# hzheng40/irbfn

Hardware: AMD Instinct MI355X
Metric: RBF-net evals/s (B queries x N centres), forward (higher is better)
Workload: dtype f32 (distances and Phi x W on f16 MFMA: exact fixed-point heads + float tails, hi/lo operand pairs; f32 accumulate)

## Files before the change

### irbfn_amd/csrc/abi.hip

```cpp
#include <new>
#include <string.h>

#include "common.h"
#include "rollout_step.h"

namespace irbfn {
thread_local int g_last_hip_error = 0;
int padded_D(int D);
}

using namespace irbfn;

static inline hipStream_t as_stream(void* s) { return reinterpret_cast<hipStream_t>(s); }

extern "C" {

int irbfn_abi_version(void) { return IRBFN_ABI_VERSION; }

int irbfn_last_hip_error(void) { return g_last_hip_error; }

int irbfn_device_count(void) {
  int n = 0;
  hipError_t e = hipGetDeviceCount(&n);
  if (e != hipSuccess) {
// ... 31 lines not shown
  if (DC < 0 || OP < 0) return IRBFN_ERR_UNSUPPORTED;
  for (int i = 0; i < n_ranges * nsplit; ++i)
    if (dim_ranges_host[i] < 0 || dim_ranges_host[i] >= max_ranges) return IRBFN_ERR_BAD_ARG;
  if (n_ranges > R) n_ranges = R;

  irbfn_net* net = new (std::nothrow) irbfn_net();
  if (!net) return IRBFN_ERR_BAD_ARG;
  memset(net, 0, sizeof(*net));
  net->D = D; net->R = R; net->K = K; net->O = O; net->basis = basis;
  net->bclass = basis_class(basis);
  net->DC = DC; net->OP = OP; net->N = R * K;
  net->S = (DC + 1 + OP + 3) & ~3;
  net->nsplit = nsplit; net->max_ranges = max_ranges > 0 ? max_ranges : 1; net->n_ranges = n_ranges;
  net->opt[IRBFN_OPT_FWD_F16_TERMS] = 3;
  net->opt[IRBFN_OPT_TICK_FUSED] = 1;

  const size_t tab = (size_t)(nsplit > 0 ? nsplit : 1) * net->max_ranges;
  const size_t nr = (size_t)(n_ranges > 0 ? n_ranges : 1) * (nsplit > 0 ? nsplit : 1);
  hipError_t e = hipSuccess;
  auto alloc = [&](void** p, size_t bytes) {
    if (e == hipSuccess) e = hipMalloc(p, bytes ? bytes : 4);
  };
  alloc((void**)&net->rec, (size_t)net->N * net->S * sizeof(float));
  alloc((void**)&net->bias, (size_t)OP * sizeof(float));
  alloc((void**)&net->sig2, (size_t)net->N * sizeof(float));
  net->Npad = (net->N + 15) & ~15;
  if (mfma_eligible(net)) alloc((void**)&net->recm, (size_t)net->Npad * mfma_record_floats(D, O) * sizeof(float));
  if (f16_eligible(net)) {
    alloc((void**)&net->f16_img, f16_image_bytes(net));
    alloc((void**)&net->f16_oscale, 128 * sizeof(float));
// ... 351 lines not shown
```

### irbfn_amd/csrc/common.h

```cpp
#pragma once

#include <hip/hip_runtime.h>
#include <stdint.h>

#include "irbfn_hip.h"

namespace irbfn {

constexpr int kWave = 64;
constexpr int kMaxSplit = 8;
constexpr int kMaxD = 8;
constexpr int kRedBlocks = 256;
constexpr int kSeedBlocksMax = 1024;

enum BasisClass : int { BC_GAUSS = 0, BC_IQ = 1, BC_IMQ = 2, BC_GENERIC = 3 };

inline int basis_class(int basis) {
  switch (basis) {
    case IRBFN_GAUSSIAN:
    case IRBFN_GAUSSIAN_WIDE:
    case IRBFN_GAUSSIAN_WIDER: return BC_GAUSS;
    case IRBFN_INVERSE_QUADRATIC: return BC_IQ;
    case IRBFN_INVERSE_MULTIQUADRIC: return BC_IMQ;
    default: return BC_GENERIC;
// ... 9 lines not shown
#define IRBFN_HIP_CHECK(expr)                         \
  do {                                                \
    hipError_t e__ = (expr);                          \
    if (e__ != hipSuccess) {                          \
      ::irbfn::g_last_hip_error = (int)e__;           \
      return IRBFN_ERR_HIP;                           \
    }                                                 \
  } while (0)

struct GateTables {
  const float* lo;
  const float* hi;
  const float* delta;
  const int* dim_ranges;
  int nsplit, max_ranges, n_ranges;
};

__host__ __device__ constexpr int mfma_cw(int D) { return (D + 1 + 3) & ~3; }

struct DynParams {
  float p[13];
};
struct DynParams64 {
  double p[13];
};
template <typename S> struct DynOf { using type = DynParams; };
template <> struct DynOf<double> { using type = DynParams64; };

}

// ... 14 lines not shown
  void* gram_hdr;
  int gram_ok;
  int gram_exp[5];
  int gram_checked;
  float* pack_part;
  int gamma_packed;
  int* vjp_flags;
  int vjp_gen;
  float* small_part;
  unsigned int* small_ticket;
  float* gate_lo;
  float* gate_hi;
  float* gate_delta;
  int* gate_ranges;
  int nsplit, max_ranges, n_ranges;
  float* sp_img;
  int sp_ok, sp_E, sp_cap, sp_RS, sp_EW, sp_OPS;
  float sp_mean_active;
  bool has_params;
  int opt[IRBFN_OPT_COUNT];
  char last_name[96];
  int last_grid, last_block;

  irbfn::GateTables gate() const {
    return irbfn::GateTables{gate_lo, gate_hi, gate_delta, gate_ranges, nsplit, max_ranges, n_ranges};
  }
};

namespace irbfn {
enum LaunchKind : int {
// ... 150 lines not shown
```

### irbfn_amd/csrc/rbf_forward.hip

```cpp
#include <math.h>
#include "rbf_forward.h"
#include "rollout_step.h"

#include <stdio.h>
#include <stdlib.h>
#include <string.h>

namespace irbfn {

int launch_forward_d3(const FwdArgs&, int, int, int, bool, bool, int, size_t, hipStream_t, int*);
int launch_forward_d4(const FwdArgs&, int, int, int, bool, bool, int, size_t, hipStream_t, int*);
int launch_forward_d7(const FwdArgs&, int, int, int, bool, bool, int, size_t, hipStream_t, int*);
int launch_forward_d8(const FwdArgs&, int, int, int, bool, bool, int, size_t, hipStream_t, int*);

static const int kCompiledOP[] = {2, 4, 5, 8, 10, 16, 32, 64, 100, 128};

int padded_O(int O) {
  for (int op : kCompiledOP)
    if (O <= op) return op;
  return -1;
}

int padded_D(int D) {
  if (D <= 3) return 3;
// ... 217 lines not shown

static void gram_wide_geometry(const irbfn_net* net, int64_t B, int* SW_out, int* QG_out) {
  const int nchunks = (net->N + 31) / 32;
  const long groups = (B + 31) / 32;
  int SW = 1;
  while (SW < 4 && (groups * SW + 7) / 8 < 256) SW *= 2;
  SW = opt_or(net, IRBFN_OPT_FWD_F16_S, SW);
  if (SW != 1 && SW != 2 && SW != 4) SW = 1;
  while (SW > 1 && (gram_wide_ring_bytes(net, SW) > 160 * 1024 || nchunks / SW < 2)) SW /= 2;
  int QG = groups <= 384 ? 2 : (SW == 1 ? 4 : 8 / SW);
  QG = opt_or(net, IRBFN_OPT_FWD_F16_QG, QG);
  if (QG < 1 || SW * QG > 8) QG = 8 / SW;
  *SW_out = SW; *QG_out = QG;
}

static bool plan_gram(const irbfn_net* net, int64_t B, LaunchPlan* p) {
  if (!net->f16_img || !gram_eligible(net)) return false;
  int S, QG;
  size_t lds;
  if (net->O > 16) {
    if ((net->DC != 7 && net->DC != 8) || net->O > 128) return false;
    gram_wide_geometry(net, B, &S, &QG);
    lds = gram_wide_lds_bytes(net, S, QG, 0);
    p->kind = LK_K1G_WIDE;
  } else {
    gram_geometry(net, B, (net->N + 31) / 32, &S, &QG);
    lds = gram_lds_bytes(S, QG, false);
    p->kind = LK_K1G;
  }
  if (lds > 160 * 1024) {
    p->kind = LK_NONE;
    return false;
  }
  p->status = IRBFN_OK;
  p->S = S; p->QG = QG; p->lds = lds;
  p->grid = (int)(((B + 31) / 32 + QG - 1) / QG); p->block = S * QG * 64;
  return true;
}

static LaunchPlan plan_forward(const irbfn_net* net, int64_t B) {
  LaunchPlan p;
// ... 190 lines not shown
  LaunchPlan p;
  if (!gram_gamma_eligible(net)) return p;
  const bool packed = net->gram_img && net->f16_img && (net->R == 1 || net->gamma_packed);
  if (!packed) { p.status = IRBFN_ERR_NO_PARAMS; return p; }
  if (!net->gram_ok) return p;
  const int nchunks = net->R * gram_gamma_cpr(net);
  int S, QG;
  gram_geometry(net, B, nchunks, &S, &QG);
  const int fs = net->opt[IRBFN_OPT_FWD_F16_S];
  if (fs > 0 && fs <= 7 && S != fs) {
    S = fs;
    QG = opt_or(net, IRBFN_OPT_FWD_F16_QG, 8 / S > 0 ? 8 / S : 1);
    if (S * QG > 16) QG = 1;
  }
  p.lds = gram_lds_bytes(S, QG, tick, true);
  if (p.lds > 160 * 1024) return p;
  p.kind = tick ? LK_TICK_K1G_GAMMA : LK_K1G_GAMMA; p.status = IRBFN_OK; p.mode = mode;
  p.S = S; p.QG = QG;
  p.grid = (int)(((B + 31) / 32 + QG - 1) / QG); p.block = S * QG * 64;
  return p;
}

int launch_forward_gamma(irbfn_net* net, const float* x, const float* gamma, float* out, int64_t B, hipStream_t s) {
  if (B == 0) return IRBFN_OK;
  if (net->opt[IRBFN_OPT_FWD_GAMMA_KERNEL] == IRBFN_FWDG_K1G) {
    const LaunchPlan g = plan_gram_gamma(net, B, false, -1);
    if (g.kind == LK_NONE) return g.status;
    const int rc = launch_forward_gram_gamma(net, g, x, gamma, out, B, s);
    if (rc == IRBFN_OK) record_launch(net, g);
    return rc;
  }
// ... 101 lines not shown
```

### irbfn_amd/csrc/rbf_forward_f16_narrow.h

```cpp
#pragma once

#include "rbf_forward_f16_wide.h"

namespace irbfn {

constexpr int kTickNarrowT = 8;
constexpr int kTickNarrowCP = 17;
constexpr int kTickNarrowSP = 65;

template <bool ROLL>
__device__ __forceinline__ void narrow_epilogue(const F16Args& a, const F16Roll& rl, int mode, unsigned char* lds, const f4_t (&acc)[2],
                                                const float (&gam)[2], int S, int slice, int qg, long q0, float inv_scale) {
  const int lane = threadIdx.x & 63;
  const int g = lane >> 4, n = lane & 15;
  __syncthreads();
  float* red = reinterpret_cast<float*>(lds);
  float* gl = red + (size_t)a.QG * S * 2 * 4 * 64;
  [[maybe_unused]] float* ctile = gl + a.QG * 32;
#pragma unroll
  for (int t = 0; t < 2; ++t)
#pragma unroll
    for (int r = 0; r < 4; ++r) red[(((qg * S + slice) * 2 + t) * 4 + r) * 64 + lane] = acc[t][r];
  if (slice == 0 && g == 0) { gl[qg * 32 + n] = gam[0]; gl[qg * 32 + 16 + n] = gam[1]; }
  __syncthreads();
  if (slice == 0 && n < a.O) {
    const float sc = a.oscale[n] * inv_scale;
    const float bi = a.bias[n];
#pragma unroll
    for (int t = 0; t < 2; ++t)
#pragma unroll
      for (int r = 0; r < 4; ++r) {
        float v = 0.0f;
        for (int s2 = 0; s2 < S; ++s2) v += red[(((qg * S + s2) * 2 + t) * 4 + r) * 64 + lane];
        const int row = t * 16 + 4 * g + r;
        const long q = q0 + row;
        float y = __builtin_fmaf(gl[qg * 32 + row] * v, sc, bi);
        if constexpr (ROLL) {
          if (rl.mirror != nullptr && n >= rl.T && q < a.B && rl.mirror[q] != 0) y = -y;
          ctile[(qg * 32 + row) * kTickNarrowCP + n] = y;
        }
        if (q < a.B && a.out != nullptr) a.out[q * a.O + n] = y;
      }
// ... 9 lines not shown
    float u[2 * kTickNarrowT];
    if (lane < 32) {
      const float* ur = ctile + (qg * 32 + lane) * kTickNarrowCP;
#pragma unroll
      for (int i = 0; i < 2 * kTickNarrowT; ++i) u[i] = ur[i];
    }
    asm volatile("s_waitcnt lgkmcnt(0)" ::: "memory");
    __builtin_amdgcn_wave_barrier();
    float* stage = ctile + (size_t)a.QG * 32 * kTickNarrowCP + (size_t)qg * 32 * kTickNarrowSP;
    if (lane < nvalid) {
      const long b = q0 + lane;
      float* o = stage + lane * kTickNarrowSP;
      auto ctl = [&](int i) {
        float v = u[0];
#pragma unroll
        for (int k = 1; k < 2 * kTickNarrowT; ++k) v = (i == k) ? u[k] : v;
        return v;
      };
      if (mode == IRBFN_ROLLOUT_ST_SELECT || mode == IRBFN_ROLLOUT_ST_KS) {
        float st[7];
#pragma unroll
        for (int i = 0; i < 7; ++i) st[i] = rl.state0[b * 7 + i];
        for (int t = 0; t < T; ++t) {
          if (mode == IRBFN_ROLLOUT_ST_SELECT) st_step<true>(st, ctl(t), ctl(T + t), rl.dp);
          else st_step<false>(st, ctl(t), ctl(T + t), rl.dp);
#pragma unroll
          for (int i = 0; i < 7; ++i) o[t * 7 + i] = st[i];
        }
      } else if (mode == IRBFN_ROLLOUT_FRENET_LS) {
        float st[8];
#pragma unroll
// ... 28 lines not shown
```

### irbfn_amd/csrc/rbf_forward_gram.h

```cpp
#pragma once

#include "rbf_forward_f16_narrow.h"

namespace irbfn {

typedef _Float16 h4_t __attribute__((ext_vector_type(4)));

constexpr int kGramHeadBytes = 2 * 64 * 8;
constexpr int kGramTailBytes = 2 * 2 * 64 * 16;
constexpr int kGramOpBytes = kGramHeadBytes + kGramTailBytes;
constexpr int gram_chunk_bytes(int NT = 1) { return kGramOpBytes + NT * 2 * kF16WBytes; }
constexpr int kGramChunkBytes = gram_chunk_bytes(1);
constexpr int kGramDims = 8;
#ifndef IRBFN_GRAM_RING
#define IRBFN_GRAM_RING 5
#endif
constexpr int kGramRing = IRBFN_GRAM_RING;
#ifndef IRBFN_GRAM_WAVES
#define IRBFN_GRAM_WAVES 4
#endif

struct GramHdr {
  float r[8];
  int ex, ec, eq, ea, e2;
// ... 15 lines not shown
  const int m = hf * 3 + (j - 5);
  return j < 5 ? GramSlot{1, 2 * g + hf, gram_comb_p(j), gram_comb_q(j)}
               : (g == 0 ? (m < 5 ? GramSlot{2, 0, gram_comb_p(m), gram_comb_q(m)} : GramSlot{3, 0, 2, 0})
                         : (g == 1 && hf == 0 && j == 5 ? GramSlot{3, 0, 3, 0} : GramSlot{0, 0, 0, 0}));
}
static_assert(kGramDims == 8, "four lane groups x two coordinates");
__host__ __device__ inline int gram_T(const GramHdr& h, const GramSlot sl) {
  return sl.kind == 1 ? h.ex + h.ec - 11 * (sl.p + sl.q) : (sl.kind == 2 ? h.eq + h.ea - 11 * (sl.p + sl.q) : h.e2 - 11 * sl.p);
}
__host__ __device__ inline int gram_ax(int T) { return (T + 1) >> 1; }

template <int BC>
__host__ __device__ constexpr float gram_phi_scale() { return BC == BC_IMQ ? 128.0f : kPhiScale; }

#ifdef IRBFN_GRAM_STAMPS
__device__ unsigned long long g_gram_stamps[32];
#define IRBFN_GRAM_T() __builtin_amdgcn_s_memtime()
#else
#define IRBFN_GRAM_T() 0ull
#endif

typedef float f2_t __attribute__((ext_vector_type(2)));
typedef unsigned u2_t __attribute__((ext_vector_type(2)));

__device__ __forceinline__ void split_pair_mix(float p0, float p1, unsigned& hi, unsigned& lo) {
  hi = __builtin_bit_cast(unsigned, __builtin_amdgcn_cvt_pkrtz(p0, p1));
  const float q0 = p0 * kLoGain, q1 = p1 * kLoGain;
  const float ng = -kLoGain;
  float d0, d1;
  asm("v_fma_mix_f32 %0, %1, %2, %3 op_sel:[0,0,0] op_sel_hi:[1,0,0]" : "=v"(d0) : "v"(hi), "s"(ng), "v"(q0));
  asm("v_fma_mix_f32 %0, %1, %2, %3 op_sel:[1,0,0] op_sel_hi:[1,0,0]" : "=v"(d1) : "v"(hi), "s"(ng), "v"(q1));
  lo = __builtin_bit_cast(unsigned, __builtin_amdgcn_cvt_pkrtz(d0, d1));
}

template <int BC>
// ... 7 lines not shown
                 "v"(u[T][1][2]), "v"(u[T][1][3]));
#define IRBFN_T8_TAIL0 ""
#define IRBFN_T8_TAIL1 "\n s_nop 7"
  if constexpr (BC == BC_GAUSS) { IRBFN_T8("v_exp_f32_e32", 0) IRBFN_T8("v_exp_f32_e32", 1) }
  else if constexpr (BC == BC_IQ) { IRBFN_T8("v_rcp_f32_e32", 0) IRBFN_T8("v_rcp_f32_e32", 1) }
  else { IRBFN_T8("v_rsq_f32_e32", 0) IRBFN_T8("v_rsq_f32_e32", 1) }
#undef IRBFN_T8
#undef IRBFN_T8_TAIL0
#undef IRBFN_T8_TAIL1
}

struct GramArgs {
  F16Args f;
  const unsigned char* __restrict__ gimg;
  const GramHdr* __restrict__ hdr;
};

__device__ __forceinline__ void gram_parts_f(float vh, float vl, float inv, float (&n)[3]) {
  const float a = vh * inv, b = vl * inv;
  n[0] = __builtin_rintf(a * 1024.0f) * (1.0f / 1024.0f);
  const float r1 = ((a - n[0]) + b) * 2048.0f;
  n[1] = (float)(_Float16)r1;
  const float r2 = (r1 - n[1]) * 2048.0f;
  n[2] = (float)(_Float16)r2;
}

template <int DC>
__device__ __forceinline__ bool gram_query_operands(const F16Args& a, const GramHdr* hp, const long (&qrow)[2], int g, h4_t (&bhd)[2],
                                                    h8_t (&btl)[2][2]) {
#pragma clang fp contract(off)
  static_assert(DC <= kGramDims, "eight coordinate slots");
  const int ex = hp->ex, ec = hp->ec, eq = hp->eq, ea = hp->ea, e2 = hp->e2;
  GramHdr hx;
  hx.ex = ex; hx.ec = ec; hx.eq = eq; hx.ea = ea; hx.e2 = e2;
  bool bad = hp->ok == 0;
  const float xinv = __builtin_ldexpf(1.0f, -ex), qinv = __builtin_ldexpf(1.0f, -eq);
  const float xlim = __builtin_ldexpf(1.0f, ex) * 0.999f, qlim = __builtin_ldexpf(1.0f, eq) * 0.999f;
  auto scale_of = [&](const GramSlot sl) -> float { return sl.kind == 0 ? 0.0f : __builtin_ldexpf(1.0f, gram_ax(gram_T(hx, sl))); };
  float rr[2];
#pragma unroll
  for (int c = 0; c < 2; ++c) rr[c] = (2 * g + c < DC) ? -hp->r[2 * g + c] : 0.0f;
#pragma unroll
  for (int t = 0; t < 2; ++t) {
    float nx[2][3], nq[3];
    float qh = 0.0f, ql = 0.0f;
#pragma unroll
    for (int c = 0; c < 2; ++c) {
      const int i = 2 * g + c;
      const float xv = (i < DC && i < a.Dreal) ? a.x[qrow[t] * a.Dreal + i] : 0.0f;
      const float sh = xv + rr[c];
      const float bb = sh - xv;
      const float sl = (xv - (sh - bb)) + (rr[c] - bb);
      bad = bad || !(__builtin_fabsf(sh) < xlim);
      gram_parts_f(sh, sl, xinv, nx[c]);
      const float ph = sh * sh;
      const float pl = __builtin_fmaf(sh, sh, -ph) + 2.0f * sh * sl;
      const float th = qh + ph;
      const float tb = th - qh;
      ql += ((qh - (th - tb)) + (ph - tb)) + pl;
      qh = th;
    }
#pragma unroll
    for (int off = 16; off <= 32; off *= 2) {
      const float oh = __shfl_xor(qh, off), ol = __shfl_xor(ql, off);
// ... 19 lines not shown
      for (int j = 0; j < 5; ++j) {
        const GramSlot sl = gram_tail_slot(32 * hf + j);
        btl[t][hf][j] = (_Float16)(nx[hf][sl.p] * scale_of(sl));
      }
#pragma unroll
      for (int j = 5; j < 8; ++j) {
        const GramSlot s0 = gram_tail_slot(32 * hf + j), s1 = gram_tail_slot(32 * hf + 8 + j);
        const float v0 = s0.kind == 2 ? nq[s0.p] * scale_of(s0) : scale_of(s0);
        const float v1 = scale_of(s1);
        btl[t][hf][j] = (_Float16)(g == 0 ? v0 : (g == 1 ? v1 : 0.0f));
      }
    }
  }
  return bad;
}
static_assert(gram_head_slot(0).kind == 1 && gram_head_slot(4 * 3 + 1).dim == 7 && gram_head_slot(2).kind == 2 && gram_head_slot(6).kind == 3 &&
              gram_head_slot(10).kind == 3 && gram_head_slot(10).p == 1 && gram_head_slot(14).kind == 0 && gram_head_slot(3).kind == 0, "head slots");
static_assert(gram_tail_slot(32 + 8 * 2 + 4).kind == 1 && gram_tail_slot(32 + 8 * 2 + 4).dim == 5 && gram_tail_slot(5).kind == 2 &&
              gram_tail_slot(32 + 6).kind == 2 && gram_tail_slot(32 + 7).kind == 3 && gram_tail_slot(32 + 7).p == 2 && gram_tail_slot(8 + 5).kind == 3 &&
              gram_tail_slot(8 + 5).p == 3 && gram_tail_slot(8 + 6).kind == 0 && gram_tail_slot(16 + 5).kind == 0 && gram_tail_slot(32 + 8 + 5).kind == 0, "tail slots");

__device__ __forceinline__ void gram_heads(const h4_t (&a)[2], const h4_t (&b)[2], f4_t (&u)[2][2]) {
  asm("v_mfma_f32_16x16x16_f16 %0, %4, %6, 0\n v_mfma_f32_16x16x16_f16 %1, %5, %6, 0\n v_mfma_f32_16x16x16_f16 %2, %4, %7, 0\n "
      "v_mfma_f32_16x16x16_f16 %3, %5, %7, 0\n s_nop 4"
      : "=&v"(u[0][0]), "=&v"(u[0][1]), "=&v"(u[1][0]), "=&v"(u[1][1])
      : "v"(a[0]), "v"(a[1]), "v"(b[0]), "v"(b[1]));
}
__device__ __forceinline__ void gram_heads2(const h4_t& a, const h4_t (&b)[2], f4_t (&u)[2]) {
  asm("v_mfma_f32_16x16x16_f16 %0, %2, %3, 0\n v_mfma_f32_16x16x16_f16 %1, %2, %4, 0\n s_nop 4"
      : "=&v"(u[0]), "=&v"(u[1])
// ... 39 lines not shown
      const float* rp = recs + ((j >> 2) * 16 + 4 * g + (j & 3)) * RF;
      float r2 = 0.0f;
#pragma unroll
      for (int d = 0; d < DC; ++d) {
        const float df = xq[d] - rp[d];
        r2 = __builtin_fmaf(df, df, r2);
      }
      if constexpr (FINITE_R2) r2 = r2 == __builtin_inff() ? 3.0e38f : r2;
      float arg = f16_arg<BC>(r2, rp[RF - 1]);
      if constexpr (BC == BC_IMQ) arg *= kPhiScale;
      t16[t * 8 + j] = arg;
    }
  }
}

void gram_fill_args(const irbfn_net* net, const float* x, float* out, int64_t B, int S, int QG, GramArgs* a);
int launch_forward_gram_wide(irbfn_net* net, const LaunchPlan& p, const float* x, float* out, int64_t B, hipStream_t s);

}
```

### irbfn_amd/csrc/rbf_forward_gram.hip

```cpp
#include <hip/hip_fp16.h>
#include <stdint.h>
#include <stdio.h>
#include <stdlib.h>

#include "rbf_forward_gram_body.h"

namespace irbfn {

template <int DC, int BC>
__global__ __launch_bounds__(1024, IRBFN_GRAM_WAVES) void rbf_fwd_f16gram(const GramArgs ga) {
  extern __shared__ __attribute__((aligned(16))) unsigned char lds[];
  gram_body<DC, BC, false>(ga, F16Roll{}, -1, lds);
}

template <int DC, int BC>
__global__ __launch_bounds__(1024, IRBFN_GRAM_WAVES) void rbf_tick_f16gram(const GramArgs ga, const F16Roll rl, const int mode) {
  extern __shared__ __attribute__((aligned(16))) unsigned char lds[];
  gram_body<DC, BC, true>(ga, rl, mode, lds);
}

static int gram_nt(const irbfn_net* net) { return (net->O + 15) / 16; }

bool gram_eligible(const irbfn_net* net) {
  return f16_eligible(net) && net->DC <= kGramDims;
}

size_t gram_image_bytes(const irbfn_net* net) {
  const int nchunks = (net->N + kF16Chunk - 1) / kF16Chunk;
  return (size_t)nchunks * gram_chunk_bytes(gram_nt(net));
}

size_t gram_header_bytes() { return sizeof(GramHdr); }

#ifdef IRBFN_GRAM_STAMPS
extern "C" int irbfn_debug_gram_stamps(unsigned long long* out32) {
  return (int)hipMemcpyFromSymbol(out32, HIP_SYMBOL(g_gram_stamps), sizeof(unsigned long long) * 32);
}
#endif

template <int DC>
static int launch_gram_bc(const GramArgs& a, int bc, int grid, int block, size_t lds, hipStream_t s) {
#define IRBFN_GCASE(BCV)                                                                                      \
  case BCV: {                                                                                                 \
    auto k = rbf_fwd_f16gram<DC, BCV>;                                                                        \
    if (lds > 48 * 1024) {                                                                                    \
      hipError_t e = hipFuncSetAttribute(reinterpret_cast<const void*>(k),                                    \
                                         hipFuncAttributeMaxDynamicSharedMemorySize, (int)lds);               \
      if (e != hipSuccess) { g_last_hip_error = (int)e; return IRBFN_ERR_HIP; }                               \
    }                                                                                                         \
    hipLaunchKernelGGL(k, dim3(grid), dim3(block), lds, s, a);                                                \
    break;                                                                                                    \
  }
  switch (bc) {
    IRBFN_GCASE(BC_GAUSS)
    IRBFN_GCASE(BC_IQ)
    IRBFN_GCASE(BC_IMQ)
    default: return IRBFN_ERR_UNSUPPORTED;
  }
#undef IRBFN_GCASE
  IRBFN_HIP_CHECK(hipGetLastError());
  return IRBFN_OK;
}

size_t gram_lds_bytes(int S, int QG, bool tick, bool gamma) {
  size_t ring = (size_t)S * kGramRing * kGramChunkBytes;
  if (gamma) ring += (size_t)S * QG * 128 * sizeof(float);
  size_t red = (size_t)S * QG * 2 * 4 * 64 + (size_t)QG * 32;
  if (tick) red += (size_t)QG * 32 * (kTickNarrowCP + kTickNarrowSP);
  red *= sizeof(float);
  return ring > red ? ring : red;
}

int launch_forward_gram(irbfn_net* net, const LaunchPlan& p, const float* x, float* out, int64_t B, hipStream_t s) {
  if (p.kind == LK_K1G_WIDE) return launch_forward_gram_wide(net, p, x, out, B, s);
  GramArgs a;
  gram_fill_args(net, x, out, B, p.S, p.QG, &a);
  switch (net->DC) {
    case 3: return launch_gram_bc<3>(a, net->bclass, p.grid, p.block, p.lds, s);
    case 4: return launch_gram_bc<4>(a, net->bclass, p.grid, p.block, p.lds, s);
    case 7: return launch_gram_bc<7>(a, net->bclass, p.grid, p.block, p.lds, s);
    case 8: return launch_gram_bc<8>(a, net->bclass, p.grid, p.block, p.lds, s);
    default: return IRBFN_ERR_UNSUPPORTED;
  }
}

template <int DC>
static int launch_tick_gram_bc(const GramArgs& a, const F16Roll& rl, int mode, int bc, int grid, int block, size_t lds, hipStream_t s) {
#define IRBFN_GCASE(BCV)                                                                                      \
  case BCV: {                                                                                                 \
    auto k = rbf_tick_f16gram<DC, BCV>;                                                                       \
    if (lds > 48 * 1024) {                                                                                    \
      hipError_t e = hipFuncSetAttribute(reinterpret_cast<const void*>(k),                                    \
                                         hipFuncAttributeMaxDynamicSharedMemorySize, (int)lds);               \
      if (e != hipSuccess) { g_last_hip_error = (int)e; return IRBFN_ERR_HIP; }                               \
    }                                                                                                         \
    hipLaunchKernelGGL(k, dim3(grid), dim3(block), lds, s, a, rl, mode);                                      \
    break;                                                                                                    \
  }
  switch (bc) {
    IRBFN_GCASE(BC_GAUSS)
    IRBFN_GCASE(BC_IQ)
    IRBFN_GCASE(BC_IMQ)
    default: return IRBFN_ERR_UNSUPPORTED;
  }
#undef IRBFN_GCASE
  IRBFN_HIP_CHECK(hipGetLastError());
  return IRBFN_OK;
}

int launch_tick_gram_narrow(irbfn_net* net, const LaunchPlan& p, const float* x, const int* mirror, const float* state0,
// ... 11 lines not shown
```

### irbfn_amd/csrc/rbf_forward_gram_body.h

```cpp
#pragma once

#include "rbf_forward_gram.h"

namespace irbfn {

struct GramGamma {
  const float* __restrict__ gamma;
  int R, cpr;
};

template <int DC, int BC, bool ROLL, bool GAMMA = false>
__device__ __forceinline__ void gram_body(const GramArgs& ga, const F16Roll& rl, int mode, unsigned char* lds,
                                          [[maybe_unused]] const GramGamma gm = GramGamma{nullptr, 1, 1}) {
  static_assert(DC <= kGramDims, "eight coordinate slots");
  const F16Args& a = ga.f;
  constexpr int CBL = f16_chunk_bytes(DC);
  constexpr int CB = kGramChunkBytes;
  const int tid = threadIdx.x, lane = tid & 63;
  const int wave = __builtin_amdgcn_readfirstlane(tid >> 6);
  const int S = a.S, QG = a.QG;
  const int slice = wave / QG, qg = wave % QG;
  const int g = lane >> 4, n = lane & 15;
  const long q0 = ((long)blockIdx.x * QG + qg) * 32;
  const GramHdr* hp = ga.hdr;
  long qrow[2];
#pragma unroll
  for (int t = 0; t < 2; ++t) {
    long q = q0 + t * 16 + n;
    q = q < a.B ? q : a.B - 1;
    qrow[t] = q < 0 ? 0 : q;
  }
  h4_t bhd[2];
  h8_t btl[2][2];
  const bool bad = gram_query_operands<DC>(a, hp, qrow, g, bhd, btl);
  const bool wave_bad = __builtin_amdgcn_ballot_w64(bad) != 0ull;

  const int c0 = (int)((long)a.nchunks * slice / S), c1 = (int)((long)a.nchunks * (slice + 1) / S);
  const int na = c1 - c0;
  int nsteps = 0;
  for (int s2 = 0; s2 < S; ++s2) {
    const int m = (int)((long)a.nchunks * (s2 + 1) / S) - (int)((long)a.nchunks * s2 / S);
    nsteps = m > nsteps ? m : nsteps;
  }
  unsigned char* ring = lds + (size_t)slice * kGramRing * CB;
  constexpr int NVI = CB / 1024;
  auto stage = [&](int k, int buf) {
    if (k >= na) return;
    const unsigned char* gp = ga.gimg + (size_t)(c0 + k) * CB + lane * 16;
    unsigned char* dst = ring + buf * CB;
    for (int v = qg; v < NVI; v += QG)
      __builtin_amdgcn_global_load_lds((gptr_t)(gp + v * 1024), (lptr_t)(dst + v * 1024), 16, 0, 0);
  };
  auto step_barrier = [&]() { asm volatile("s_waitcnt vmcnt(0) lgkmcnt(0)\n\ts_barrier" ::: "memory"); };
  auto next3 = [&](int b3) { return b3 == kGramRing - 1 ? 0 : b3 + 1; };
  constexpr int kGramPer = (kGramRing - 1) / 2;
  static_assert(kGramRing == 2 * kGramPer + 1 && kGramPer >= 1, "ring = 2 x (steps per barrier) + 1");
  [[maybe_unused]] float* gtile = nullptr;
  [[maybe_unused]] const float* grow = nullptr;
// ... 54 lines not shown
      unsigned wh[4], wl[4];
#pragma unroll
      for (int jj = 0; jj < 4; ++jj) split_pair_mix(t16[t * 8 + 2 * jj], t16[t * 8 + 2 * jj + 1], wh[jj], wl[jj]);
      const h8_t ah = __builtin_bit_cast(h8_t, u4_t{wh[0], wh[1], wh[2], wh[3]});
      const h8_t al = __builtin_bit_cast(h8_t, u4_t{wl[0], wl[1], wl[2], wl[3]});
      acc[t] = __builtin_amdgcn_mfma_f32_16x16x32_f16(ah, bh, acc[t], 0, 0, 0);
      acl[t] = __builtin_amdgcn_mfma_f32_16x16x32_f16(al, bh, acl[t], 0, 0, 0);
      acl[t] = __builtin_amdgcn_mfma_f32_16x16x32_f16(ah, bl, acl[t], 0, 0, 0);
    }
  };

#pragma unroll
  for (int k = 0; k <= kGramPer; ++k) stage(k, k);
  gamma_stage(0);
  step_barrier();
#pragma unroll
  for (int k = kGramPer + 1; k < kGramRing; ++k) stage(k, k);
  gamma_stage(1);
  if (!wave_bad) {
    f4_t ua[2][2], ub[2][2];
    if (na > 0) distances(ring, ua);
    asm volatile("s_nop 7\n\ts_nop 7" ::: "memory");
    int b0 = 0;
    [[maybe_unused]] unsigned long long tph[5] = {0, 0, 0, 0, 0};
    auto one_step = [&](int i, f4_t (&ucur)[2][2], f4_t (&unxt)[2][2]) {
      const int b1 = next3(b0);
      [[maybe_unused]] const unsigned long long t0 = IRBFN_GRAM_T();
      if (i + 1 < na) distances(ring + b1 * CB, unxt);
      if (i < na) {
        gamma_read(i);
        float t16[16];
        products(t16, ring + b0 * CB, [&](float (&o)[16]) { trans16<BC>(ucur, o); });
      }
      [[maybe_unused]] const unsigned long long t2 = IRBFN_GRAM_T();
      end_of_step(i, b0);
      [[maybe_unused]] const unsigned long long t4 = IRBFN_GRAM_T();
#ifdef IRBFN_GRAM_STAMPS
      tph[1] += t2 - t0; tph[2] += t4 - t2; tph[4] += 1;
#endif
      b0 = b1;
    };
    for (int i = 0; i < nsteps; i += 2) {
      one_step(i, ua, ub);
      if (i + 1 < nsteps) one_step(i + 1, ub, ua);
    }
#ifdef IRBFN_GRAM_STAMPS
    if (blockIdx.x < 2 && tid == 0)
      for (int k = 0; k < 5; ++k) g_gram_stamps[blockIdx.x * 8 + k] = tph[k];
#endif
  } else {
    int b0 = 0;
    for (int i = 0; i < nsteps; ++i) {
      if (i < na) {
        gamma_read(i);
        float t16[16];
        gram_valu_args<DC, BC, GAMMA>(a, qrow, g, reinterpret_cast<const float*>(a.img + (size_t)(c0 + i) * CBL), t16);
        products(t16, ring + b0 * CB, [&](float (&o)[16]) { trans_block<BC, 16>(o); });
      }
      end_of_step(i, b0);
      b0 = next3(b0);
    }
  }
#pragma unroll
  for (int t = 0; t < 2; ++t)
#pragma unroll
    for (int r = 0; r < 4; ++r) acc[t][r] = __builtin_fmaf(acl[t][r], kLoScale, acc[t][r]);

  const GateTables gt = a.gate;
  float gam[2] = {0.0f, 0.0f};
  if constexpr (GAMMA) {
    gam[0] = gam[1] = 1.0f;
  } else if (slice == 0) {
#pragma unroll
    for (int t = 0; t < 2; ++t) {
      float gv = gt.n_ranges > 0 ? 1.0f : 0.0f;
#pragma unroll
      for (int d = 0; d < DC; ++d)
        if (d < gt.nsplit && gt.n_ranges > 0) {
          const int e = d * gt.max_ranges + gt.dim_ranges[d];
          gv *= gate_factor(a.x[qrow[t] * a.Dreal + d], gt.lo[e], gt.hi[e], gt.delta[d]);
        }
      gam[t] = gv;
    }
  }
  narrow_epilogue<ROLL>(a, rl, mode, lds, acc, gam, S, slice, qg, q0, 1.0f / (gram_phi_scale<BC>() * kWScale));
}

}
```

### irbfn_amd/csrc/rbf_forward_gram_gamma.hip

```cpp
#ifdef IRBFN_GRAM_STAMPS
#undef IRBFN_GRAM_STAMPS
#endif
#include <hip/hip_fp16.h>
#include <stdint.h>

#include "rbf_forward_gram_body.h"

namespace irbfn {

template <int DC, int BC>
__global__ __launch_bounds__(1024, IRBFN_GRAM_WAVES) void rbf_fwd_f16gram_gamma(const GramArgs ga, const GramGamma gm) {
  extern __shared__ __attribute__((aligned(16))) unsigned char lds[];
  gram_body<DC, BC, false, true>(ga, F16Roll{}, -1, lds, gm);
}

template <int DC, int BC>
__global__ __launch_bounds__(1024, IRBFN_GRAM_WAVES) void rbf_tick_f16gram_gamma(const GramArgs ga, const GramGamma gm, const F16Roll rl,
                                                                                 const int mode) {
  extern __shared__ __attribute__((aligned(16))) unsigned char lds[];
  gram_body<DC, BC, true, true>(ga, rl, mode, lds, gm);
}

int gram_gamma_cpr(const irbfn_net* net) { return (net->K + kF16Chunk - 1) / kF16Chunk; }

// ... 17 lines not shown
  }
  net->f16_img = static_cast<unsigned char*>(bufs[0]);
  net->f16_oscale = static_cast<float*>(bufs[1]);
  net->gram_img = static_cast<unsigned char*>(bufs[2]);
  net->gram_hdr = bufs[3];
  net->pack_part = static_cast<float*>(bufs[4]);
  net->gamma_packed = 0;
  return IRBFN_OK;
}

static void gamma_fill_args(const irbfn_net* net, const float* x, const float* gamma, float* out, int64_t B, int S, int QG, GramArgs* a,
                            GramGamma* gm) {
  gram_fill_args(net, x, out, B, S, QG, a);
  gm->gamma = gamma; gm->R = net->R; gm->cpr = gram_gamma_cpr(net);
  a->f.nchunks = gm->R * gm->cpr;
}

template <typename K, typename... Args>
static int launch_gg(K k, int grid, int block, size_t lds, hipStream_t s, Args... args) {
  if (lds > 48 * 1024) {
    hipError_t e = hipFuncSetAttribute(reinterpret_cast<const void*>(k), hipFuncAttributeMaxDynamicSharedMemorySize, (int)lds);
    if (e != hipSuccess) { g_last_hip_error = (int)e; return IRBFN_ERR_HIP; }
  }
  hipLaunchKernelGGL(k, dim3(grid), dim3(block), lds, s, args...);
  IRBFN_HIP_CHECK(hipGetLastError());
  return IRBFN_OK;
}

template <int DC>
static int launch_gg_fwd(const GramArgs& a, const GramGamma& gm, int bc, const LaunchPlan& p, hipStream_t s) {
// ... 44 lines not shown
```

### irbfn_amd/csrc/rbf_forward_gram_wide.hip

```cpp
#include "rbf_forward_gram_wide.h"

namespace irbfn {

template <int DC, int BC, int NT>
__global__ __launch_bounds__(512) void rbf_fwd_f16gram_wide(const GramArgs ga) {
  extern __shared__ __attribute__((aligned(16))) unsigned char lds[];
  wide_gram_body<DC, BC, NT, -1>(ga, F16Roll{}, lds);
}

template <int DC, int NT>
static int launch_gw_bc(const GramArgs& a, int bc, int grid, int block, size_t lds, hipStream_t s) {
#define IRBFN_GWCASE(BCV)                                                                                     \
  case BCV: {                                                                                                 \
    auto k = rbf_fwd_f16gram_wide<DC, BCV, NT>;                                                                \
    if (lds > 48 * 1024) {                                                                                    \
      hipError_t e = hipFuncSetAttribute(reinterpret_cast<const void*>(k),                                    \
                                         hipFuncAttributeMaxDynamicSharedMemorySize, (int)lds);               \
      if (e != hipSuccess) { g_last_hip_error = (int)e; return IRBFN_ERR_HIP; }                               \
    }                                                                                                         \
    hipLaunchKernelGGL(k, dim3(grid), dim3(block), lds, s, a);                                                \
    break;                                                                                                    \
  }
  switch (bc) {
    IRBFN_GWCASE(BC_GAUSS)
// ... 2 lines not shown
    default: return IRBFN_ERR_UNSUPPORTED;
  }
#undef IRBFN_GWCASE
  IRBFN_HIP_CHECK(hipGetLastError());
  return IRBFN_OK;
}

size_t gram_wide_ring_bytes(const irbfn_net* net, int SW) { return (size_t)SW * 3 * gram_chunk_bytes((net->O + 15) / 16); }

size_t gram_wide_lds_bytes(const irbfn_net* net, int SW, int QG, size_t extra_red_floats) {
  const size_t ring = gram_wide_ring_bytes(net, SW);
  const size_t red = ((size_t)SW * QG * 2 * 4 * 64 + (size_t)QG * 32 + extra_red_floats) * sizeof(float);
  return ring > red ? ring : red;
}

void gram_fill_args(const irbfn_net* net, const float* x, float* out, int64_t B, int S, int QG, GramArgs* a) {
  const int nchunks = (net->N + kF16Chunk - 1) / kF16Chunk;
  a->f.x = x; a->f.img = net->f16_img; a->f.oscale = net->f16_oscale; a->f.bias = net->bias; a->f.out = out; a->f.gate = net->gate();
  a->f.B = (long)B; a->f.Dreal = net->D; a->f.O = net->O; a->f.nchunks = nchunks; a->f.S = S; a->f.QG = QG;
  a->gimg = net->gram_img;
  a->hdr = reinterpret_cast<const GramHdr*>(net->gram_hdr);
}

int launch_forward_gram_wide(irbfn_net* net, const LaunchPlan& p, const float* x, float* out, int64_t B, hipStream_t s) {
  const int NT = (net->O + 15) / 16;
  GramArgs a;
  gram_fill_args(net, x, out, B, p.S, p.QG, &a);
  int rc;
#define IRBFN_GW_NT(DCV)                                                                      \
  switch (NT) {                                                                               \
    case 2: rc = launch_gw_bc<DCV, 2>(a, net->bclass, p.grid, p.block, p.lds, s); break;      \
    case 3: rc = launch_gw_bc<DCV, 3>(a, net->bclass, p.grid, p.block, p.lds, s); break;      \
    case 4: rc = launch_gw_bc<DCV, 4>(a, net->bclass, p.grid, p.block, p.lds, s); break;      \
    case 5: rc = launch_gw_bc<DCV, 5>(a, net->bclass, p.grid, p.block, p.lds, s); break;      \
    case 6: rc = launch_gw_bc<DCV, 6>(a, net->bclass, p.grid, p.block, p.lds, s); break;      \
    case 7: rc = launch_gw_bc<DCV, 7>(a, net->bclass, p.grid, p.block, p.lds, s); break;      \
// ... 10 lines not shown
```

Measured before the change: 827.4 million.

## Hoist gram kernel prologue work: precomputed gate row, nsteps, early loads, cached LDS attr

The host now resolves the per-dimension gate bounds into a flat GateRow and precomputes nsteps, passing both as kernel arguments. That replaces the dependent global-table lookups and the per-thread loop over slices. Query and radius loads are issued early, and slice 0 computes the gate and parks it in LDS before the main loop, so the epilogue no longer waits on global reads. Other changes: an unrolled compare replaces an integer divide, bias/oscale loads move before the epilogue barrier, and the hipFuncSetAttribute call is cached per device. The cost is extra LDS for the parked gate values, a gate0 snapshot that ignores later changes to the dim_ranges table, and phase timestamp probes under a debug define.

Result: faster. 844.3 million, median of 6 (+2.0%).

```diff
diff --git a/irbfn_amd/csrc/abi.hip b/irbfn_amd/csrc/abi.hip
--- a/irbfn_amd/csrc/abi.hip
+++ b/irbfn_amd/csrc/abi.hip
@@ -69,6 +69,13 @@
   net->nsplit = nsplit; net->max_ranges = max_ranges > 0 ? max_ranges : 1; net->n_ranges = n_ranges;
   net->opt[IRBFN_OPT_FWD_F16_TERMS] = 3;
   net->opt[IRBFN_OPT_TICK_FUSED] = 1;
+
+  net->gate0.nsplit = nsplit; net->gate0.n_ranges = n_ranges;
+  if (nsplit > 0 && n_ranges > 0)
+    for (int d = 0; d < nsplit; ++d) {
+      const int e = d * net->max_ranges + dim_ranges_host[d];
+      net->gate0.lo[d] = lo_tab_host[e]; net->gate0.hi[d] = hi_tab_host[e]; net->gate0.delta[d] = delta_host[d];
+    }
 
   const size_t tab = (size_t)(nsplit > 0 ? nsplit : 1) * net->max_ranges;
   const size_t nr = (size_t)(n_ranges > 0 ? n_ranges : 1) * (nsplit > 0 ? nsplit : 1);
diff --git a/irbfn_amd/csrc/common.h b/irbfn_amd/csrc/common.h
--- a/irbfn_amd/csrc/common.h
+++ b/irbfn_amd/csrc/common.h
@@ -47,6 +47,11 @@
   const float* delta;
   const int* dim_ranges;
   int nsplit, max_ranges, n_ranges;
+};
+
+struct GateRow {
+  float lo[kMaxSplit], hi[kMaxSplit], delta[kMaxSplit];
+  int nsplit, n_ranges;
 };
 
 __host__ __device__ constexpr int mfma_cw(int D) { return (D + 1 + 3) & ~3; }
@@ -91,6 +96,7 @@
   float* gate_delta;
   int* gate_ranges;
   int nsplit, max_ranges, n_ranges;
+  irbfn::GateRow gate0;
   float* sp_img;
   int sp_ok, sp_E, sp_cap, sp_RS, sp_EW, sp_OPS;
   float sp_mean_active;
diff --git a/irbfn_amd/csrc/rbf_forward.hip b/irbfn_amd/csrc/rbf_forward.hip
--- a/irbfn_amd/csrc/rbf_forward.hip
+++ b/irbfn_amd/csrc/rbf_forward.hip
@@ -255,6 +255,8 @@
   *SW_out = SW; *QG_out = QG;
 }
 
+static bool gram_slices_fit(int nchunks, int S) { return (long)nchunks * S < (1L << 31); }
+
 static bool plan_gram(const irbfn_net* net, int64_t B, LaunchPlan* p) {
   if (!net->f16_img || !gram_eligible(net)) return false;
   int S, QG;
@@ -266,6 +268,7 @@
     p->kind = LK_K1G_WIDE;
   } else {
     gram_geometry(net, B, (net->N + 31) / 32, &S, &QG);
+    if (!gram_slices_fit((net->N + 31) / 32, S)) return false;
     lds = gram_lds_bytes(S, QG, false);
     p->kind = LK_K1G;
   }
@@ -486,7 +489,7 @@
     if (S * QG > 16) QG = 1;
   }
   p.lds = gram_lds_bytes(S, QG, tick, true);
-  if (p.lds > 160 * 1024) return p;
+  if (p.lds > 160 * 1024 || !gram_slices_fit(nchunks, S)) return p;
   p.kind = tick ? LK_TICK_K1G_GAMMA : LK_K1G_GAMMA; p.status = IRBFN_OK; p.mode = mode;
   p.S = S; p.QG = QG;
   p.grid = (int)(((B + 31) / 32 + QG - 1) / QG); p.block = S * QG * 64;
diff --git a/irbfn_amd/csrc/rbf_forward_f16_narrow.h b/irbfn_amd/csrc/rbf_forward_f16_narrow.h
--- a/irbfn_amd/csrc/rbf_forward_f16_narrow.h
+++ b/irbfn_amd/csrc/rbf_forward_f16_narrow.h
@@ -13,6 +13,11 @@
                                                 const float (&gam)[2], int S, int slice, int qg, long q0, float inv_scale) {
   const int lane = threadIdx.x & 63;
   const int g = lane >> 4, n = lane & 15;
+  float sc = 0.0f, bi = 0.0f;
+  if (slice == 0 && n < a.O) {
+    sc = a.oscale[n] * inv_scale;
+    bi = a.bias[n];
+  }
   __syncthreads();
   float* red = reinterpret_cast<float*>(lds);
   float* gl = red + (size_t)a.QG * S * 2 * 4 * 64;
@@ -24,8 +29,6 @@
   if (slice == 0 && g == 0) { gl[qg * 32 + n] = gam[0]; gl[qg * 32 + 16 + n] = gam[1]; }
   __syncthreads();
   if (slice == 0 && n < a.O) {
-    const float sc = a.oscale[n] * inv_scale;
-    const float bi = a.bias[n];
 #pragma unroll
     for (int t = 0; t < 2; ++t)
 #pragma unroll
@@ -65,7 +68,11 @@
       auto ctl = [&](int i) {
         float v = u[0];
 #pragma unroll
-        for (int k = 1; k < 2 * kTickNarrowT; ++k) v = (i == k) ? u[k] : v;
+        for (int k = 1; k < 2 * kTickNarrowT; ++k) {
+          float uk = u[k];
+          asm("" : "+v"(uk));
+          v = (i == k) ? uk : v;
+        }
         return v;
       };
       if (mode == IRBFN_ROLLOUT_ST_SELECT || mode == IRBFN_ROLLOUT_ST_KS) {
diff --git a/irbfn_amd/csrc/rbf_forward_gram.h b/irbfn_amd/csrc/rbf_forward_gram.h
--- a/irbfn_amd/csrc/rbf_forward_gram.h
+++ b/irbfn_amd/csrc/rbf_forward_gram.h
@@ -53,11 +53,21 @@
 __host__ __device__ constexpr float gram_phi_scale() { return BC == BC_IMQ ? 128.0f : kPhiScale; }
 
 #ifdef IRBFN_GRAM_STAMPS
-__device__ unsigned long long g_gram_stamps[32];
+__device__ unsigned long long g_gram_stamps[64];
 #define IRBFN_GRAM_T() __builtin_amdgcn_s_memtime()
+#define IRBFN_GRAM_PHASE(k)                                                                            \
+  do {                                                                                                 \
+    asm volatile("s_waitcnt vmcnt(0) lgkmcnt(0)" ::: "memory");                                        \
+    if (blockIdx.x < 2 && threadIdx.x == 0) {                                                          \
+      g_gram_stamps[blockIdx.x * 32 + 8 + (k)] = __builtin_amdgcn_s_memtime();                         \
+      if ((k) == 0 || (k) == 6) g_gram_stamps[blockIdx.x * 32 + 16 + (k) / 6] = __builtin_amdgcn_s_memrealtime(); \
+    }                                                                                                  \
+  } while (0)
 #else
 #define IRBFN_GRAM_T() 0ull
+#define IRBFN_GRAM_PHASE(k) do { } while (0)
 #endif
+enum GramPhase : int { GP_ENTRY = 0, GP_OPERANDS, GP_BARRIER1, GP_LOOP0, GP_LOOP1, GP_GATE, GP_STORED };
 
 typedef float f2_t __attribute__((ext_vector_type(2)));
 typedef unsigned u2_t __attribute__((ext_vector_type(2)));
@@ -95,6 +105,8 @@
   F16Args f;
   const unsigned char* __restrict__ gimg;
   const GramHdr* __restrict__ hdr;
+  GateRow g0;
+  int nsteps;
 };
 
 __device__ __forceinline__ void gram_parts_f(float vh, float vl, float inv, float (&n)[3]) {
@@ -107,8 +119,24 @@
 }
 
 template <int DC>
-__device__ __forceinline__ bool gram_query_operands(const F16Args& a, const GramHdr* hp, const long (&qrow)[2], int g, h4_t (&bhd)[2],
-                                                    h8_t (&btl)[2][2]) {
+__device__ __forceinline__ void gram_query_loads(const F16Args& a, const GramHdr* hp, const long (&qrow)[2], int g, float (&xv)[2][2],
+                                                 float (&rv)[2]) {
+#pragma unroll
+  for (int c = 0; c < 2; ++c) rv[c] = hp->r[2 * g + c];
+#pragma unroll
+  for (int t = 0; t < 2; ++t)
+#pragma unroll
+    for (int c = 0; c < 2; ++c) {
+      const int i = 2 * g + c;
+      const bool in = i < DC && i < a.Dreal;
+      const float v = a.x[qrow[t] * a.Dreal + (in ? i : 0)];
+      xv[t][c] = in ? v : 0.0f;
+    }
+}
+
+template <int DC>
+__device__ __forceinline__ bool gram_query_operands(const F16Args& a, const GramHdr* hp, const float (&xin)[2][2], const float (&rin)[2],
+                                                    int g, h4_t (&bhd)[2], h8_t (&btl)[2][2]) {
 #pragma clang fp contract(off)
   static_assert(DC <= kGramDims, "eight coordinate slots");
   const int ex = hp->ex, ec = hp->ec, eq = hp->eq, ea = hp->ea, e2 = hp->e2;
@@ -120,15 +148,16 @@
   auto scale_of = [&](const GramSlot sl) -> float { return sl.kind == 0 ? 0.0f : __builtin_ldexpf(1.0f, gram_ax(gram_T(hx, sl))); };
   float rr[2];
 #pragma unroll
-  for (int c = 0; c < 2; ++c) rr[c] = (2 * g + c < DC) ? -hp->r[2 * g + c] : 0.0f;
+  for (int c = 0; c < 2; ++c) {
+    rr[c] = (2 * g + c < DC) ? -rin[c] : 0.0f;
+  }
 #pragma unroll
   for (int t = 0; t < 2; ++t) {
     float nx[2][3], nq[3];
     float qh = 0.0f, ql = 0.0f;
 #pragma unroll
     for (int c = 0; c < 2; ++c) {
-      const int i = 2 * g + c;
-      const float xv = (i < DC && i < a.Dreal) ? a.x[qrow[t] * a.Dreal + i] : 0.0f;
+      const float xv = xin[t][c];
       const float sh = xv + rr[c];
       const float bb = sh - xv;
       const float sl = (xv - (sh - bb)) + (rr[c] - bb);
@@ -178,6 +207,13 @@
   }
   return bad;
 }
+template <int DC>
+__device__ __forceinline__ bool gram_query_operands(const F16Args& a, const GramHdr* hp, const long (&qrow)[2], int g, h4_t (&bhd)[2],
+                                                    h8_t (&btl)[2][2]) {
+  float xv[2][2], rv[2];
+  gram_query_loads<DC>(a, hp, qrow, g, xv, rv);
+  return gram_query_operands<DC>(a, hp, xv, rv, g, bhd, btl);
+}
 static_assert(gram_head_slot(0).kind == 1 && gram_head_slot(4 * 3 + 1).dim == 7 && gram_head_slot(2).kind == 2 && gram_head_slot(6).kind == 3 &&
               gram_head_slot(10).kind == 3 && gram_head_slot(10).p == 1 && gram_head_slot(14).kind == 0 && gram_head_slot(3).kind == 0, "head slots");
 static_assert(gram_tail_slot(32 + 8 * 2 + 4).kind == 1 && gram_tail_slot(32 + 8 * 2 + 4).dim == 5 && gram_tail_slot(5).kind == 2 &&
@@ -247,6 +283,7 @@
   }
 }
 
+int gram_nsteps(int nchunks, int S);
 void gram_fill_args(const irbfn_net* net, const float* x, float* out, int64_t B, int S, int QG, GramArgs* a);
 int launch_forward_gram_wide(irbfn_net* net, const LaunchPlan& p, const float* x, float* out, int64_t B, hipStream_t s);
 
diff --git a/irbfn_amd/csrc/rbf_forward_gram.hip b/irbfn_amd/csrc/rbf_forward_gram.hip
--- a/irbfn_amd/csrc/rbf_forward_gram.hip
+++ b/irbfn_amd/csrc/rbf_forward_gram.hip
@@ -3,9 +3,13 @@
 #include <stdio.h>
 #include <stdlib.h>
 
+#include <atomic>
+
 #include "rbf_forward_gram_body.h"
 
 namespace irbfn {
+
+constexpr int kMaxDevices = 64;
 
 template <int DC, int BC>
 __global__ __launch_bounds__(1024, IRBFN_GRAM_WAVES) void rbf_fwd_f16gram(const GramArgs ga) {
@@ -33,21 +37,29 @@
 size_t gram_header_bytes() { return sizeof(GramHdr); }
 
 #ifdef IRBFN_GRAM_STAMPS
-extern "C" int irbfn_debug_gram_stamps(unsigned long long* out32) {
-  return (int)hipMemcpyFromSymbol(out32, HIP_SYMBOL(g_gram_stamps), sizeof(unsigned long long) * 32);
+extern "C" int irbfn_debug_gram_stamps(unsigned long long* out64) {
+  return (int)hipMemcpyFromSymbol(out64, HIP_SYMBOL(g_gram_stamps), sizeof(unsigned long long) * 64);
 }
 #endif
+
+struct DynLdsSet { std::atomic<unsigned> bytes[kMaxDevices]; };
+static int ensure_dyn_lds(const void* kernel, size_t lds, DynLdsSet* set) {
+  if (lds <= 48 * 1024) return IRBFN_OK;
+  int dev = 0;
+  IRBFN_HIP_CHECK(hipGetDevice(&dev));
+  if (dev >= 0 && dev < kMaxDevices && set->bytes[dev].load(std::memory_order_relaxed) >= lds) return IRBFN_OK;
+  IRBFN_HIP_CHECK(hipFuncSetAttribute(kernel, hipFuncAttributeMaxDynamicSharedMemorySize, (int)lds));
+  if (dev >= 0 && dev < kMaxDevices) set->bytes[dev].store((unsigned)lds, std::memory_order_relaxed);
+  return IRBFN_OK;
+}
 
 template <int DC>
 static int launch_gram_bc(const GramArgs& a, int bc, int grid, int block, size_t lds, hipStream_t s) {
 #define IRBFN_GCASE(BCV)                                                                                      \
   case BCV: {                                                                                                 \
     auto k = rbf_fwd_f16gram<DC, BCV>;                                                                        \
-    if (lds > 48 * 1024) {                                                                                    \
-      hipError_t e = hipFuncSetAttribute(reinterpret_cast<const void*>(k),                                    \
-                                         hipFuncAttributeMaxDynamicSharedMemorySize, (int)lds);               \
-      if (e != hipSuccess) { g_last_hip_error = (int)e; return IRBFN_ERR_HIP; }                               \
-    }                                                                                                         \
+    static DynLdsSet set;                                                                                     \
+    if (const int rc = ensure_dyn_lds(reinterpret_cast<const void*>(k), lds, &set); rc != IRBFN_OK) return rc; \
     hipLaunchKernelGGL(k, dim3(grid), dim3(block), lds, s, a);                                                \
     break;                                                                                                    \
   }
@@ -65,6 +77,7 @@
 size_t gram_lds_bytes(int S, int QG, bool tick, bool gamma) {
   size_t ring = (size_t)S * kGramRing * kGramChunkBytes;
   if (gamma) ring += (size_t)S * QG * 128 * sizeof(float);
+  else ring += (size_t)QG * 32 * sizeof(float);
   size_t red = (size_t)S * QG * 2 * 4 * 64 + (size_t)QG * 32;
   if (tick) red += (size_t)QG * 32 * (kTickNarrowCP + kTickNarrowSP);
   red *= sizeof(float);
@@ -89,11 +102,8 @@
 #define IRBFN_GCASE(BCV)                                                                                      \
   case BCV: {                                                                                                 \
     auto k = rbf_tick_f16gram<DC, BCV>;                                                                       \
-    if (lds > 48 * 1024) {                                                                                    \
-      hipError_t e = hipFuncSetAttribute(reinterpret_cast<const void*>(k),                                    \
-                                         hipFuncAttributeMaxDynamicSharedMemorySize, (int)lds);               \
-      if (e != hipSuccess) { g_last_hip_error = (int)e; return IRBFN_ERR_HIP; }                               \
-    }                                                                                                         \
+    static DynLdsSet set;                                                                                     \
+    if (const int rc = ensure_dyn_lds(reinterpret_cast<const void*>(k), lds, &set); rc != IRBFN_OK) return rc; \
     hipLaunchKernelGGL(k, dim3(grid), dim3(block), lds, s, a, rl, mode);                                      \
     break;                                                                                                    \
   }
diff --git a/irbfn_amd/csrc/rbf_forward_gram_body.h b/irbfn_amd/csrc/rbf_forward_gram_body.h
--- a/irbfn_amd/csrc/rbf_forward_gram_body.h
+++ b/irbfn_amd/csrc/rbf_forward_gram_body.h
@@ -17,9 +17,13 @@
   constexpr int CBL = f16_chunk_bytes(DC);
   constexpr int CB = kGramChunkBytes;
   const int tid = threadIdx.x, lane = tid & 63;
+  IRBFN_GRAM_PHASE(GP_ENTRY);
   const int wave = __builtin_amdgcn_readfirstlane(tid >> 6);
   const int S = a.S, QG = a.QG;
-  const int slice = wave / QG, qg = wave % QG;
+  int slice = 0;
+#pragma unroll
+  for (int s2 = 1; s2 < 8; ++s2) slice += wave >= s2 * QG ? 1 : 0;
+  const int qg = wave - slice * QG;
   const int g = lane >> 4, n = lane & 15;
   const long q0 = ((long)blockIdx.x * QG + qg) * 32;
   const GramHdr* hp = ga.hdr;
@@ -30,18 +34,40 @@
     q = q < a.B ? q : a.B - 1;
     qrow[t] = q < 0 ? 0 : q;
   }
+  float xop[2][2], rop[2];
+  gram_query_loads<DC>(a, hp, qrow, g, xop, rop);
+  [[maybe_unused]] float* gpark = reinterpret_cast<float*>(lds + (size_t)S * kGramRing * CB) + qg * 32;
+  if constexpr (!GAMMA) {
+    if (slice == 0) {
+      const GateRow& gr = ga.g0;
+      float xg[2][DC];
+#pragma unroll
+      for (int t = 0; t < 2; ++t)
+#pragma unroll
+        for (int d = 0; d < DC; ++d) xg[t][d] = a.x[qrow[t] * a.Dreal + (d < gr.nsplit ? d : 0)];
+#pragma unroll
+      for (int t = 0; t < 2; ++t) {
+        float gv = gr.n_ranges > 0 ? 1.0f : 0.0f;
+#pragma unroll
+        for (int d = 0; d < DC; ++d)
+          if (d < gr.nsplit && gr.n_ranges > 0) gv *= gate_factor(xg[t][d], gr.lo[d], gr.hi[d], gr.delta[d]);
+        if (g == 0) gpark[t * 16 + n] = gv;
+      }
+    }
+  }
   h4_t bhd[2];
   h8_t btl[2][2];
-  const bool bad = gram_query_operands<DC>(a, hp, qrow, g, bhd, btl);
-  const bool wave_bad = __builtin_amdgcn_ballot_w64(bad) != 0ull;
-
-  const int c0 = (int)((long)a.nchunks * slice / S), c1 = (int)((long)a.nchunks * (slice + 1) / S);
+  const bool bad = gram_query_operands<DC>(a, hp, xop, rop, g, bhd, btl);
+  const bool wave_bad = __builtin_amdgcn_readfirstlane(__builtin_amdgcn_ballot_w64(bad) != 0ull ? 1 : 0) != 0;
+#ifdef IRBFN_GRAM_STAMPS
+  asm volatile("" ::"s"((int)wave_bad), "v"(bhd[1]), "v"(btl[1][1]));
+#endif
+  IRBFN_GRAM_PHASE(GP_OPERANDS);
+
+  const unsigned nch = (unsigned)a.nchunks;
+  const int c0 = (int)(nch * (unsigned)slice / (unsigned)S), c1 = (int)(nch * (unsigned)(slice + 1) / (unsigned)S);
   const int na = c1 - c0;
-  int nsteps = 0;
-  for (int s2 = 0; s2 < S; ++s2) {
-    const int m = (int)((long)a.nchunks * (s2 + 1) / S) - (int)((long)a.nchunks * s2 / S);
-    nsteps = m > nsteps ? m : nsteps;
-  }
+  const int nsteps = ga.nsteps;
   unsigned char* ring = lds + (size_t)slice * kGramRing * CB;
   constexpr int NVI = CB / 1024;
   auto stage = [&](int k, int buf) {
@@ -126,9 +152,11 @@
   for (int k = 0; k <= kGramPer; ++k) stage(k, k);
   gamma_stage(0);
   step_barrier();
+  IRBFN_GRAM_PHASE(GP_BARRIER1);
 #pragma unroll
   for (int k = kGramPer + 1; k < kGramRing; ++k) stage(k, k);
   gamma_stage(1);
+  IRBFN_GRAM_PHASE(GP_LOOP0);
   if (!wave_bad) {
     f4_t ua[2][2], ub[2][2];
     if (na > 0) distances(ring, ua);
@@ -158,7 +186,7 @@
     }
 #ifdef IRBFN_GRAM_STAMPS
     if (blockIdx.x < 2 && tid == 0)
-      for (int k = 0; k < 5; ++k) g_gram_stamps[blockIdx.x * 8 + k] = tph[k];
+      for (int k = 0; k < 5; ++k) g_gram_stamps[blockIdx.x * 32 + k] = tph[k];
 #endif
   } else {
     int b0 = 0;
@@ -173,29 +201,25 @@
       b0 = next3(b0);
     }
   }
+  IRBFN_GRAM_PHASE(GP_LOOP1);
 #pragma unroll
   for (int t = 0; t < 2; ++t)
 #pragma unroll
     for (int r = 0; r < 4; ++r) acc[t][r] = __builtin_fmaf(acl[t][r], kLoScale, acc[t][r]);
 
-  const GateTables gt = a.gate;
   float gam[2] = {0.0f, 0.0f};
   if constexpr (GAMMA) {
     gam[0] = gam[1] = 1.0f;
   } else if (slice == 0) {
-#pragma unroll
-    for (int t = 0; t < 2; ++t) {
-      float gv = gt.n_ranges > 0 ? 1.0f : 0.0f;
-#pragma unroll
-      for (int d = 0; d < DC; ++d)
-        if (d < gt.nsplit && gt.n_ranges > 0) {
-          const int e = d * gt.max_ranges + gt.dim_ranges[d];
-          gv *= gate_factor(a.x[qrow[t] * a.Dreal + d], gt.lo[e], gt.hi[e], gt.delta[d]);
-        }
-      gam[t] = gv;
-    }
-  }
+    gam[0] = gpark[n];
+    gam[1] = gpark[16 + n];
+  }
+#ifdef IRBFN_GRAM_STAMPS
+  asm volatile("" ::"v"(gam[0]), "v"(gam[1]));
+#endif
+  IRBFN_GRAM_PHASE(GP_GATE);
   narrow_epilogue<ROLL>(a, rl, mode, lds, acc, gam, S, slice, qg, q0, 1.0f / (gram_phi_scale<BC>() * kWScale));
+  IRBFN_GRAM_PHASE(GP_STORED);
 }
 
 }
diff --git a/irbfn_amd/csrc/rbf_forward_gram_gamma.hip b/irbfn_amd/csrc/rbf_forward_gram_gamma.hip
--- a/irbfn_amd/csrc/rbf_forward_gram_gamma.hip
+++ b/irbfn_amd/csrc/rbf_forward_gram_gamma.hip
@@ -55,6 +55,7 @@
   gram_fill_args(net, x, out, B, S, QG, a);
   gm->gamma = gamma; gm->R = net->R; gm->cpr = gram_gamma_cpr(net);
   a->f.nchunks = gm->R * gm->cpr;
+  a->nsteps = gram_nsteps(a->f.nchunks, S);
 }
 
 template <typename K, typename... Args>
diff --git a/irbfn_amd/csrc/rbf_forward_gram_wide.hip b/irbfn_amd/csrc/rbf_forward_gram_wide.hip
--- a/irbfn_amd/csrc/rbf_forward_gram_wide.hip
+++ b/irbfn_amd/csrc/rbf_forward_gram_wide.hip
@@ -40,12 +40,23 @@
   return ring > red ? ring : red;
 }
 
+int gram_nsteps(int nchunks, int S) {
+  int nsteps = 0;
+  for (int s2 = 0; s2 < S; ++s2) {
+    const int m = (int)((long)nchunks * (s2 + 1) / S) - (int)((long)nchunks * s2 / S);
+    nsteps = m > nsteps ? m : nsteps;
+  }
+  return nsteps;
+}
+
 void gram_fill_args(const irbfn_net* net, const float* x, float* out, int64_t B, int S, int QG, GramArgs* a) {
   const int nchunks = (net->N + kF16Chunk - 1) / kF16Chunk;
   a->f.x = x; a->f.img = net->f16_img; a->f.oscale = net->f16_oscale; a->f.bias = net->bias; a->f.out = out; a->f.gate = net->gate();
   a->f.B = (long)B; a->f.Dreal = net->D; a->f.O = net->O; a->f.nchunks = nchunks; a->f.S = S; a->f.QG = QG;
   a->gimg = net->gram_img;
   a->hdr = reinterpret_cast<const GramHdr*>(net->gram_hdr);
+  a->g0 = net->gate0;
+  a->nsteps = gram_nsteps(nchunks, S);
 }
 
 int launch_forward_gram_wide(irbfn_net* net, const LaunchPlan& p, const float* x, float* out, int64_t B, hipStream_t s) {
```
